# firedrakeproject/firedrake

Hardware: NVIDIA H100
Metric: assembled DoFs/sec (Poisson CG3, 256^3 hex, 1-form/action) (higher is better)
Workload: dtype f64

## Files before the change

### firedrake_b200/_lib.py

```python
from __future__ import annotations

import ctypes as C
import os

HERE = os.path.dirname(os.path.abspath(__file__))
LIB_PATH = os.environ.get("FDB200_LIB", os.path.join(HERE, "lib", "libfdb200.so"))

MAX_1D = 8

FORM_HELMHOLTZ = 1
FORM_DG_ADVECTION = 2
FORM_HELMHOLTZ_COEF = 3
FORM_NONLINEAR_DIFFUSION = 4
FORM_NONLINEAR_DIFFUSION_JACOBIAN = 5
FORM_ELASTICITY = 6
FORM_HYPERELASTICITY = 7
FORM_HYPERELASTICITY_JACOBIAN = 8
FORM_ADVECTION_DIFFUSION = 9
FORM_STOKES = 10
FORM_NAVIER_STOKES = 11
FORM_NAVIER_STOKES_JACOBIAN = 12
FORM_BOUNDARY_MASS = 13
FORM_INTERIOR_PENALTY = 14
FORM_DG_BOUNDARY = 15
# ... 20 lines not shown
    _fields_ = [
        ("form", C.c_int32), ("rank", C.c_int32), ("cell", C.c_int32),
        ("integral", C.c_int32), ("degree", C.c_int32), ("nq", C.c_int32),
        ("cdim", C.c_int32), ("scatter", C.c_int32),
        ("alpha", C.c_double), ("beta", C.c_double),
        ("B", C.c_double * (MAX_1D * MAX_1D)), ("D", C.c_double * (MAX_1D * MAX_1D)),
        ("wq", C.c_double * MAX_1D), ("xq", C.c_double * MAX_1D),
        ("offset0", C.POINTER(C.c_int32)), ("offset1", C.POINTER(C.c_int32)),
        ("diagonal", C.c_int32), ("affine_cells", C.c_int32),
        ("dcoef", C.c_double * 3),
        ("lmbda", C.c_double),
    ]


class Space2Desc(C.Structure):
    _fields_ = [
        ("degree", C.c_int32),
        ("B", C.c_double * (MAX_1D * MAX_1D)),
        ("offset", C.POINTER(C.c_int32)),
    ]


class CallArgs(C.Structure):
    _fields_ = [
        ("start", C.c_int32), ("end", C.c_int32),
        ("layers", C.POINTER(C.c_int32)), ("subset", C.c_void_p),
        ("nargs", C.c_int32), ("args", C.POINTER(C.c_void_p)),
        ("arg_bytes", C.POINTER(C.c_size_t)), ("arg_versions", C.POINTER(C.c_uint64)),
        ("nmaps", C.c_int32), ("maps", C.POINTER(C.c_void_p)),
        ("map_bytes", C.POINTER(C.c_size_t)),
        ("location", C.c_int32), ("writeback", C.c_int32), ("output_is_zero", C.c_int32),
        ("map_versions", C.POINTER(C.c_uint64)), ("subset_version", C.c_uint64),
        ("layers_count", C.c_int32), ("layers_version", C.c_uint64),
    ]


READ, WRITE, RW, INC, MIN, MAX = 1, 2, 3, 4, 5, 6
ARG_DAT, ARG_GLOBAL, ARG_MAT = 1, 2, 3
F64, F32, I32, U32, I64 = 1, 2, 3, 4, 5
REGION_ALL, REGION_ON_BOTTOM, REGION_ON_TOP, REGION_ON_INTERIOR_FACETS = 0, 1, 2, 3
WRAP_MAX_ARGS, WRAP_MAX_MAPS, WRAP_MAX_MATS = 16, 8, 4


class WrapperArg(C.Structure):
    _fields_ = [
        ("kind", C.c_int32), ("access", C.c_int32), ("dtype", C.c_int32),
        ("dim", C.c_int32), ("dim2", C.c_int32), ("map", C.c_int32), ("map2", C.c_int32),
        ("arity", C.c_int32), ("arity2", C.c_int32),
        ("offset", C.POINTER(C.c_int32)), ("offset2", C.POINTER(C.c_int32)),
        ("permutation", C.POINTER(C.c_int32)),
        ("interior_horizontal", C.c_int32),
        ("offset_quotient", C.POINTER(C.c_int32)), ("offset_quotient2", C.POINTER(C.c_int32)),
        ("mixed_continuation", C.c_int32),
    ]


class WrapperDesc(C.Structure):
    _fields_ = [
        ("kernel_source", C.c_char_p), ("kernel_name", C.c_char_p),
        ("nargs", C.c_int32), ("args", C.POINTER(WrapperArg)),
        ("extruded", C.c_int32), ("subset", C.c_int32), ("iteration_region", C.c_int32),
        ("pass_layer_arg", C.c_int32), ("extruded_periodic", C.c_int32), ("variable_layers", C.c_int32),
    ]


SIGNATURES = {
# ... 134 lines not shown
```

### firedrake_b200/csrc/action_hex.cu

```cuda
#include <stdlib.h>
#include <string.h>

#include "common.cuh"

namespace {

template <int N>
struct HelmParams {
    double *y;
    const double *x;
    const double *coords;
    const int *map0;
    const int *map1;
    const int *collist;
    const int *off0;
    const int *off1;
    int ncols;
    int col0;
    int nlay_items;
    int lay_first, lay_step;
    unsigned nlay_rcp;
    int cdim;
    const long long *rowptr;
    const int *colidx;
    double *vals;
    const int *row_lg;
    const int *col_lg;
    const unsigned short *rank_tab;
    int nvar, nlay_total;
    int chunk;
    int ws_flags;
    int *counter;
    double alpha, beta;
    double B[N * N];
    double Dt[N * N];
    double DtR[N * N];
    double DB[N * N];
    double wq[N];
    double xq[N];
};

template <int N>
struct HelmCoefParams : HelmParams<N> {
    const double *kappa;
};

template <int N>
struct HelmNlParams : HelmCoefParams<N> {
    double dcoef[3];
};

template <bool COEF>
__device__ __forceinline__ double coef_weight(double w, const double *s_kap, int q)
{
    if constexpr (COEF) return w * s_kap[q];
    else return w;
}

template <bool COEF, int NL>
__device__ __forceinline__ double stiff_weight(double w, const double *s_kap, int q, double uq, const double *dcoef)
{
    if constexpr (NL == 1) return w * fma(fma(dcoef[2], uq, dcoef[1]), uq, dcoef[0]);
    else if constexpr (NL == 2) return w;
    else return coef_weight<COEF>(w, s_kap, q);
}
// ... 258 lines not shown
    constexpr int WARPS_PER_CTA = WPC<N, SLIM, COEF>::value;
    constexpr int T = WARPS_PER_CTA * 32;
    auto kern = [] {
        if constexpr (ADV) return advection_diffusion_kernel<N, MASS, ATOMIC, MINB, MATRIX>;
        else if constexpr (NL == 1) return nonlinear_residual_kernel<N, MASS, ATOMIC, MINB, SLIM>;
        else if constexpr (NL == 2) return nonlinear_jacobian_kernel<N, MASS, ATOMIC, MINB, MATRIX, SLIM>;
        else if constexpr (COEF) return helmholtz_coef_kernel<N, MASS, ATOMIC, MINB, MATRIX, SLIM>;
        else return helmholtz_action_kernel<N, MASS, ATOMIC, MINB, MATRIX, SLIM, AFFINE>;
    }();
    static bool configured = false;
    static int occ = 1;
    if (!configured) {
        FDB_CUDA(cudaFuncSetAttribute(kern, cudaFuncAttributeMaxDynamicSharedMemorySize, WS::CTA_BYTES));
        FDB_CUDA(cudaOccupancyMaxActiveBlocksPerMultiprocessor(&occ, kern, T, WS::CTA_BYTES));
        if (occ < 1) occ = 1;
        configured = true;
    }
    const int ncells = P.ncols * P.nlay_items;
    const int nitems = (ncells + WS::CW - 1) / WS::CW;
    int per_sm = occ;
    if (grid_cap_per_sm > 0 && grid_cap_per_sm < per_sm) per_sm = grid_cap_per_sm;
    long long grid = (long long)sm_count * per_sm;
    long long need = (nitems + WARPS_PER_CTA - 1) / WARPS_PER_CTA;
    if (grid > need) grid = need;
    if (grid < 1) grid = 1;
    int chunk = P.nlay_items / WS::CW;
    if (chunk < 8) chunk = 8;
    if (chunk > 64) chunk = 64;
    long long per_warp = nitems / (grid * WARPS_PER_CTA) + 1;
    if (chunk > per_warp / 32 + 1) chunk = (int)(per_warp / 32 + 1);
    static const int chunk_env = getenv("FDB_CHUNK") ? atoi(getenv("FDB_CHUNK")) : 0;
    if (chunk_env > 0) chunk = chunk_env;
    P.chunk = chunk;
    P.nlay_rcp = (unsigned)(0x100000000ull / (unsigned long long)P.nlay_items);
    if (P.nlay_items == 1) P.nlay_rcp = 0xffffffffu;
    FDB_CUDA(cudaMemsetAsync(P.counter, 0, sizeof(int), st));
    if constexpr (NL != 0) kern<<<(int)grid, T, WS::CTA_BYTES, st>>>(P);
    else if constexpr (COEF) kern<<<(int)grid, T, WS::CTA_BYTES, st>>>(static_cast<const HelmCoefParams<N> &>(P));
    else kern<<<(int)grid, T, WS::CTA_BYTES, st>>>(static_cast<const HelmParams<N> &>(P));
    FDB_LAUNCH_CHECK();
    return 0;
}

template <int N>
struct CoefMinB {
    static constexpr int value = (N >= 5) ? 1 : 2;
};

template <int N, bool ATOMIC>
int launch_coef(bool mass, int cap, cudaStream_t st, HelmNlParams<N> &P, int sm_count)
{
    constexpr int MB = CoefMinB<N>::value;
    if (N == 6 && P.nlay_items >= 32 / N) {
        if (mass) return launch_one<N, true, ATOMIC, MB, false, (N == 6), false, true>(cap, st, P, sm_count);
        return launch_one<N, false, ATOMIC, MB, false, (N == 6), false, true>(cap, st, P, sm_count);
    }
    if (mass) return launch_one<N, true, ATOMIC, MB, false, false, false, true>(cap, st, P, sm_count);
    return launch_one<N, false, ATOMIC, MB, false, false, false, true>(cap, st, P, sm_count);
}

template <int N>
struct NlResMinB {
    static constexpr int value = (N == 4) ? 3 : ((N >= 5) ? 1 : 2);
};

template <int N, bool ATOMIC>
// ... 55 lines not shown
        constexpr bool ASL = (N == 6);
        if (!ASL || P.nlay_items >= 32 / N) {
            if (mass) return launch_one<N, true, true, AB, false, ASL, true>(cap, st, P, sm_count);
            return launch_one<N, false, true, AB, false, ASL, true>(cap, st, P, sm_count);
        }
    }
    if (N == 4 && minb == 3) {
        if (mass) return launch_one<N, true, ATOMIC, (N == 4 ? 3 : 2)>(cap, st, P, sm_count);
        return launch_one<N, false, ATOMIC, (N == 4 ? 3 : 2)>(cap, st, P, sm_count);
    }
    if (N == 4 && minb == 4) {
        if (mass) return launch_one<N, true, ATOMIC, (N == 4 ? 4 : 2)>(cap, st, P, sm_count);
        return launch_one<N, false, ATOMIC, (N == 4 ? 4 : 2)>(cap, st, P, sm_count);
    }
    if (N == 4 && minb == 1) {
        if (mass) return launch_one<N, true, ATOMIC, 1>(cap, st, P, sm_count);
        return launch_one<N, false, ATOMIC, 1>(cap, st, P, sm_count);
    }
    constexpr int DEF = (N >= 5) ? 1 : 2;
    if (N == 6) {
        static const bool slim_on = !(getenv("FDB_NO_SLIM") && atoi(getenv("FDB_NO_SLIM")));
        if (slim_on && P.nlay_items >= 32 / N) {
            if (mass) return launch_one<N, true, ATOMIC, DEF, false, (N == 6)>(cap, st, P, sm_count);
            return launch_one<N, false, ATOMIC, DEF, false, (N == 6)>(cap, st, P, sm_count);
        }
    }
    if (mass) return launch_one<N, true, ATOMIC, DEF>(cap, st, P, sm_count);
    return launch_one<N, false, ATOMIC, DEF>(cap, st, P, sm_count);
}

template <int N>
int launch_n(fdb_kernel_s *k, fdb_int start, fdb_int end, int nlay, const fdb_int *subset,
             double *y, const double *coords, const double *x, const fdb_int *map0,
             const fdb_int *map1, const double *kappa)
{
    fdb::Context &c = fdb::ctx();
    HelmNlParams<N> P;
    P.kappa = kappa;
    set_dcoef(k, P);
    const int nl = nl_mode(k);
    P.y = y;
    P.x = x;
    P.coords = coords;
    P.map0 = map0;
    P.map1 = map1;
    P.off0 = k->d_off0;
    P.off1 = k->d_off1;
    P.cdim = k->desc.cdim;
    P.alpha = k->desc.alpha;
    P.beta = k->desc.beta;
    for (int i = 0; i < N * N; i++) {
        P.B[i] = k->desc.B[i];
        P.Dt[i] = k->Dt[i];
    }
    for (int q = 0; q < N; q++)
        for (int j = 0; j < N; j++) {
            P.DtR[q * N + j] = k->Dt[q * N + (j + q) % N];
            double d = 0.0;
            for (int i = 0; i < N; i++) d += k->Dt[q * N + i] * k->desc.B[i * N + j];
            P.DB[q * N + j] = d;
        }
    for (int i = 0; i < N; i++) {
        P.wq[i] = k->desc.wq[i];
        P.xq[i] = k->desc.xq[i];
    }
    const bool mass = k->desc.beta != 0.0;
    static const int minb = getenv("FDB_MINB") ? atoi(getenv("FDB_MINB")) : 3;
    static const int cap = getenv("FDB_CTAS_PER_SM") ? atoi(getenv("FDB_CTAS_PER_SM")) : 0;
    P.counter = c.work_counter;
    if (k->desc.scatter == FDB_SCATTER_ATOMIC) {
        P.collist = subset;
        P.col0 = start;
        P.ncols = end - start;
        P.nlay_items = nlay;
        P.lay_first = 0;
        P.lay_step = 1;
        if (P.ncols <= 0 || nlay <= 0) return 0;
        if (is_adv(k)) return launch_adv<N, true>(mass, cap, c.stream, P, c.sm_count);
        if (kappa && !nl) return launch_coef<N, true>(mass, cap, c.stream, P, c.sm_count);
        if (nl) return launch_nl<N, true>(nl, mass, cap, c.stream, P, c.sm_count);
        if constexpr (N == 4) {
            static const int ws = getenv("FDB_WS") ? atoi(getenv("FDB_WS")) : 0;
            if (ws && P.cdim == 1 && nlay >= 8 && !k->desc.affine_cells) {
#define FDB_WS_CASE(id, NC, NM, NS, ST)                                                            \
    if (ws == id)                                                                              \
        return mass ? launch_ws<true, NC, NM, NS, ST>(c.stream, P, c.sm_count)                 \
                    : launch_ws<false, NC, NM, NS, ST>(c.stream, P, c.sm_count);
                FDB_WS_CASE(1, 12, 4, 2, true)
                FDB_WS_CASE(2, 8, 4, 3, true)
                FDB_WS_CASE(3, 8, 4, 3, false)
                FDB_WS_CASE(4, 8, 8, 3, false)
#undef FDB_WS_CASE
            }
        }
        return launch_variant<N, true>(mass, minb, cap, c.stream, P, c.sm_count, k->desc.affine_cells != 0);
    }
    if (subset) {
        fdb::set_error("coloured scatter does not support subsets yet");
        return 1;
    }
    for (int col = 0; col < k->ncolours; col++) {
        int cbeg = k->colour_start[col], cend = k->colour_start[col + 1];
        for (int par = 0; par < (nlay > 1 ? 2 : 1); par++) {
            P.collist = k->d_colour_cols + cbeg;
            P.col0 = 0;
            P.ncols = cend - cbeg;
            P.lay_first = par;
            P.lay_step = 2;
            P.nlay_items = (nlay - par + 1) / 2;
            if (P.ncols <= 0 || P.nlay_items <= 0) continue;
            if (is_adv(k)      ? launch_adv<N, false>(mass, cap, c.stream, P, c.sm_count)
                : kappa && !nl ? launch_coef<N, false>(mass, cap, c.stream, P, c.sm_count)
                : nl         ? launch_nl<N, false>(nl, mass, cap, c.stream, P, c.sm_count)
                             : launch_variant<N, false>(mass, minb, cap, c.stream, P, c.sm_count))
                return 1;
        }
    }
    return 0;
}

template <int N>
int launch_matrix_n(fdb_kernel_s *k, fdb_int start, fdb_int end, int nlay, const fdb_int *subset,
                    fdb_mat_t mat, const double *coords, const fdb_int *map0, const fdb_int *map1,
                    double *diag_out, const double *kappa)
{
    fdb::Context &c = fdb::ctx();
    HelmNlParams<N> P;
    memset(&P, 0, sizeof(P));
    P.kappa = kappa;
    set_dcoef(k, P);
    P.coords = coords;
    P.map0 = map0;
    P.map1 = map1;
// ... 42 lines not shown
    }
    if (nl_mode(k) == 2) {
        constexpr int MB = CoefMinB<N>::value;
        if (k->desc.beta != 0.0)
            return launch_one<N, true, true, MB, true, false, false, true, 2>(0, c.stream, P, c.sm_count);
        return launch_one<N, false, true, MB, true, false, false, true, 2>(0, c.stream, P, c.sm_count);
    }
    constexpr int DEF = (N >= 5) ? 1 : 2;
    if (k->desc.beta != 0.0) return launch_one<N, true, true, DEF, true>(0, c.stream, P, c.sm_count);
    return launch_one<N, false, true, DEF, true>(0, c.stream, P, c.sm_count);
}

}

int fdb_launch_helmholtz_matrix(fdb_kernel_s *k, fdb_int start, fdb_int end, int nlay,
                                const fdb_int *subset, fdb_mat_t mat, const double *coords,
                                const fdb_int *map0, const fdb_int *map1, double *diag_out)
{
    const int dmma = fdb_opt_matrix_kernel;
    if (mat && dmma != 0 && k->n1d <= 5 && k->n1d >= (dmma == 1 ? 3 : 4))
        return fdb_launch_helmholtz_matrix_dmma(k, start, end, nlay, subset, mat, coords, map0, map1);
    switch (k->n1d) {
    case 2: return launch_matrix_n<2>(k, start, end, nlay, subset, mat, coords, map0, map1, diag_out, nullptr);
    case 3: return launch_matrix_n<3>(k, start, end, nlay, subset, mat, coords, map0, map1, diag_out, nullptr);
    case 4: return launch_matrix_n<4>(k, start, end, nlay, subset, mat, coords, map0, map1, diag_out, nullptr);
    case 5: return launch_matrix_n<5>(k, start, end, nlay, subset, mat, coords, map0, map1, diag_out, nullptr);
    }
    fdb::set_error("helmholtz matrix: degree %d not instantiated (1..4)", k->n1d - 1);
    return 1;
}

int fdb_launch_helmholtz_action(fdb_kernel_s *k, fdb_int start, fdb_int end, int nlay,
                                const fdb_int *subset, double *y, const double *coords,
                                const double *x, const fdb_int *map0, const fdb_int *map1)
{
    static const bool q1_thread = !(getenv("FDB_Q1_THREAD") && atoi(getenv("FDB_Q1_THREAD")) == 0);
    if (q1_thread && k->n1d == 2 && k->desc.cdim == 1 && k->desc.scatter == FDB_SCATTER_ATOMIC &&
        k->desc.cell == FDB_CELL_HEX_EXTRUDED && nlay >= 16)
        return fdb_launch_q1_action(k, start, end, nlay, subset, y, coords, x, map0, map1);
    static const bool q2_thread = !(getenv("FDB_Q2_THREAD") && atoi(getenv("FDB_Q2_THREAD")) == 0);
    if (q2_thread && k->n1d == 3 && k->desc.cdim == 1 && k->desc.scatter == FDB_SCATTER_ATOMIC &&
        k->desc.cell == FDB_CELL_HEX_EXTRUDED && nlay >= 16)
        return fdb_launch_q2_action(k, start, end, nlay, subset, y, coords, x, map0, map1);
    switch (k->n1d) {
    case 2: return launch_n<2>(k, start, end, nlay, subset, y, coords, x, map0, map1, nullptr);
    case 3: return launch_n<3>(k, start, end, nlay, subset, y, coords, x, map0, map1, nullptr);
    case 4: return launch_n<4>(k, start, end, nlay, subset, y, coords, x, map0, map1, nullptr);
    case 5: return launch_n<5>(k, start, end, nlay, subset, y, coords, x, map0, map1, nullptr);
    case 6: return launch_n<6>(k, start, end, nlay, subset, y, coords, x, map0, map1, nullptr);
    }
    fdb::set_error("helmholtz action: degree %d not instantiated (1..5)", k->n1d - 1);
    return 1;
}

int fdb_launch_helmholtz_coef_action(fdb_kernel_s *k, fdb_int start, fdb_int end, int nlay,
                                     const fdb_int *subset, double *y, const double *coords,
                                     const double *x, const double *kappa, const fdb_int *map0,
                                     const fdb_int *map1)
{
    switch (k->n1d) {
    case 2: return launch_n<2>(k, start, end, nlay, subset, y, coords, x, map0, map1, kappa);
    case 3: return launch_n<3>(k, start, end, nlay, subset, y, coords, x, map0, map1, kappa);
    case 4: return launch_n<4>(k, start, end, nlay, subset, y, coords, x, map0, map1, kappa);
    case 5: return launch_n<5>(k, start, end, nlay, subset, y, coords, x, map0, map1, kappa);
    case 6: return launch_n<6>(k, start, end, nlay, subset, y, coords, x, map0, map1, kappa);
    }
    fdb::set_error("helmholtz_coef action: degree %d not instantiated (1..5)", k->n1d - 1);
    return 1;
}

int fdb_launch_helmholtz_coef_matrix(fdb_kernel_s *k, fdb_int start, fdb_int end, int nlay,
                                     const fdb_int *subset, fdb_mat_t mat, const double *coords,
                                     const double *kappa, const fdb_int *map0, const fdb_int *map1,
                                     double *diag_out)
{
    switch (k->n1d) {
    case 2: return launch_matrix_n<2>(k, start, end, nlay, subset, mat, coords, map0, map1, diag_out, kappa);
    case 3: return launch_matrix_n<3>(k, start, end, nlay, subset, mat, coords, map0, map1, diag_out, kappa);
    case 4: return launch_matrix_n<4>(k, start, end, nlay, subset, mat, coords, map0, map1, diag_out, kappa);
    case 5: return launch_matrix_n<5>(k, start, end, nlay, subset, mat, coords, map0, map1, diag_out, kappa);
    }
    fdb::set_error("helmholtz_coef matrix: degree %d not instantiated (1..4)", k->n1d - 1);
// ... 3 lines not shown
```

### firedrake_b200/csrc/action_hex_body.cuh

```cuda
    static_assert(!(SLIM && MATRIX), "matrix mode keeps the per-cell index buffer");
    static_assert(!(AFFINE && MATRIX), "the affine variant exists for 1-forms only");
    static_assert(!(AFFINE && COEF), "the coefficient form has no affine variant");
    static_assert(NL != 1 || (!COEF && !MATRIX && !AFFINE), "the residual is a 1-form without a kappa buffer");
    static_assert(NL != 2 || (COEF && !AFFINE), "the Jacobian keeps u in the kappa buffer");
    static_assert(!ADV || (COEF && NL == 0 && !SLIM && !AFFINE), "b takes the coefficient layout, three times");
    using WS = WarpSmem<N, SLIM, COEF, ADV ? 3 : 1>;
    constexpr int CW = WS::CW;
    constexpr int CWS = WS::CWS;
    constexpr int ND = N * N * N;
    constexpr int US = WS::US;
    constexpr int CS = WS::CS;
    extern __shared__ __align__(16) unsigned char smem_raw[];
    const int lane = threadIdx.x & 31, warp = threadIdx.x >> 5;
    double *wbase = reinterpret_cast<double *>(smem_raw + (size_t)warp * WS::BYTES);
    double *s_tile = wbase;
    double *s_u = s_tile + WS::TILE;
    double *s_coord = s_u + WS::UBUF;
    double *s_stash = s_coord + WS::COORD;
    constexpr bool STASH = WS::STASH > 0 && !MATRIX && !AFFINE;
    double *s_kap = s_stash + WS::STASH;
    int *s_idx = reinterpret_cast<int *>(s_kap + WS::KAPPA);
    int *s_mapraw = s_idx + WS::IDX;
    int *s_vidx = s_mapraw + WS::MAPRAW;
    int *s_off0 = reinterpret_cast<int *>(smem_raw + (size_t)WPC<N, SLIM, COEF>::value * WS::BYTES);
// ... 134 lines not shown
                const int loc = j * N + t;
                const int g = SLIM ? sm[loc] + s_off0[loc] * u.layer : si[loc];
                if constexpr (ADV) {
#pragma unroll
                    for (int c = 0; c < 3; c++) cp_async8(sk + c * WS::UBUF + loc, kappa + 3ll * g + c);
                } else {
                    cp_async8(sk + loc, kappa + g);
                }
            }
        }
    };

    Unit cur{-1, 0, 0, 0, 0, false, 0, 0, 0, false};
    cur = advance(cur);
    decode(cur);
    Unit nxt = advance(cur);
    decode(nxt);
    stageA(cur);
    cp_async_commit();
    cp_async_wait<0>();
    __syncwarp();
    int ubuf = 0;
    stageB_coords(cur);
#pragma unroll
    for (int part = 0; part < N; part++) stageB_part(cur, ubuf, part);
    stageB_kappa(cur);
    stageA(nxt);
    cp_async_commit();
    double A1[3], A3[3], A6[3], c2[3], c4[3], c5[3], c7[3];
    double Gm[6], adet_c = 1.0;
#pragma unroll
    for (int i = 0; i < 6; i++) Gm[i] = 0.0;

    while (cur.item >= 0) {
        cp_async_wait<0>();
        __syncwarp();
        Unit nn = advance(nxt);
        decode(nn);

        const bool valid = cur.valid;
        const int cbuf = cur.ib;
        const double *sc = s_coord + cw * CS;
        if (cur.comp == 0) {
#pragma unroll
            for (int a = 0; a < 3; a++) {
                double X000 = sc[0 * 3 + a], X001 = sc[1 * 3 + a], X010 = sc[2 * 3 + a],
                       X011 = sc[3 * 3 + a], X100 = sc[4 * 3 + a], X101 = sc[5 * 3 + a],
                       X110 = sc[6 * 3 + a], X111 = sc[7 * 3 + a];
                if (!valid) {
                    X000 = 0; X001 = (a == 2); X010 = (a == 1); X011 = (a >= 1);
                    X100 = (a == 0); X101 = (a != 1); X110 = (a != 2); X111 = 1;
                }
                double c1 = X100 - X000;
                c2[a] = X010 - X000;
                double c3 = X001 - X000;
                c4[a] = X110 - X100 - X010 + X000;
                c5[a] = X011 - X010 - X001 + X000;
                double c6 = X101 - X100 - X001 + X000;
                c7[a] = X111 - X110 - X101 - X011 + X100 + X010 + X001 - X000;
                A1[a] = fma(c4[a], eta, c1);
                A3[a] = fma(c5[a], eta, c3);
                A6[a] = fma(c7[a], eta, c6);
            }
            if (AFFINE) {
                double r0[3], r1[3], r2[3];
                r0[0] = c2[1] * A3[2] - c2[2] * A3[1];
                r0[1] = c2[2] * A3[0] - c2[0] * A3[2];
                r0[2] = c2[0] * A3[1] - c2[1] * A3[0];
                r1[0] = A3[1] * A1[2] - A3[2] * A1[1];
                r1[1] = A3[2] * A1[0] - A3[0] * A1[2];
                r1[2] = A3[0] * A1[1] - A3[1] * A1[0];
// ... 315 lines not shown
```

### firedrake_b200/csrc/common.cuh

```cuda
#pragma once
#include <cuda_runtime.h>
#include <stdint.h>
#include <stdio.h>
#include <string.h>

#include <string>

#include "../../include/fdb200.h"

namespace fdb {

struct Context {
    bool ready = false;
    int device = -1;
    int sm_count = 0;
    cudaStream_t stream = nullptr;
    uint64_t launches = 0;
    void *flush_buf = nullptr;
    size_t flush_bytes = 0;
    double *reduce_scratch = nullptr;
    double *reduce_host = nullptr;
    int *work_counter = nullptr;
};

// ... 63 lines not shown
typedef struct fdb_mat_s *fdb_mat_t;
int fdb_mat_device_view(fdb_mat_t m, const long long **rowptr, const fdb_int **colidx, double **vals,
                        const fdb_int **row_lg, const fdb_int **col_lg);
int fdb_mat_rank_table(fdb_mat_t m, const unsigned short **rank, int *nvar);
int fdb_mat_block_size(fdb_mat_t m, int *bs);
int fdb_mat_rows(fdb_mat_t m, fdb_int *nrows);
int fdb_mat_scalar_view_begin(fdb_mat_t blocked, fdb_mat_t *view);
int fdb_mat_scalar_view_end(fdb_mat_t blocked, fdb_mat_t view);
int fdb_launch_helmholtz_matrix(fdb_kernel_s *k, fdb_int start, fdb_int end, int nlay,
                                const fdb_int *subset, fdb_mat_t mat, const double *coords,
                                const fdb_int *map0, const fdb_int *map1, double *diag_out);

int fdb_launch_helmholtz_matrix_dmma(fdb_kernel_s *k, fdb_int start, fdb_int end, int nlay,
                                     const fdb_int *subset, fdb_mat_t mat, const double *coords,
                                     const fdb_int *map0, const fdb_int *map1);

int fdb_launch_tri_p1(fdb_kernel_s *k, fdb_int start, fdb_int end, const fdb_int *subset, double *y,
                      const double *coords, const double *x, const fdb_int *map, fdb_mat_t mat);
int fdb_launch_dg_advection(fdb_kernel_s *k, fdb_int start, fdb_int end, const fdb_int *subset,
                            double *out, const double *coords, const double *q, const double *u,
                            const double *consts_host, const unsigned *facet, const fdb_int *dgmap,
                            const fdb_int *cgmap, const fdb_int *nbr);

int fdb_launch_q1_action(fdb_kernel_s *k, fdb_int start, fdb_int end, int nlay, const fdb_int *subset,
                         double *y, const double *coords, const double *x, const fdb_int *map0,
                         const fdb_int *map1);

int fdb_launch_q2_action(fdb_kernel_s *k, fdb_int start, fdb_int end, int nlay, const fdb_int *subset,
                         double *y, const double *coords, const double *x, const fdb_int *map0,
                         const fdb_int *map1);

int fdb_launch_helmholtz_action(fdb_kernel_s *k, fdb_int start, fdb_int end, int nlay,
                                const fdb_int *subset, double *y, const double *coords,
                                const double *x, const fdb_int *map0, const fdb_int *map1);
int fdb_launch_helmholtz_coef_action(fdb_kernel_s *k, fdb_int start, fdb_int end, int nlay,
                                     const fdb_int *subset, double *y, const double *coords,
                                     const double *x, const double *kappa, const fdb_int *map0,
                                     const fdb_int *map1);
int fdb_launch_helmholtz_coef_matrix(fdb_kernel_s *k, fdb_int start, fdb_int end, int nlay,
                                     const fdb_int *subset, fdb_mat_t mat, const double *coords,
                                     const double *kappa, const fdb_int *map0, const fdb_int *map1,
                                     double *diag_out);
int fdb_launch_elasticity_action(fdb_kernel_s *k, fdb_int start, fdb_int end, int nlay, const fdb_int *subset,
                                 double *y, const double *coords, const double *x, const double *u,
                                 const fdb_int *map0, const fdb_int *map1);
int fdb_launch_elasticity_matrix(fdb_kernel_s *k, fdb_int start, fdb_int end, int nlay, const fdb_int *subset,
                                 fdb_mat_t mat, const double *coords, const double *u, const fdb_int *map0,
                                 const fdb_int *map1, double *diag_out);
int fdb_launch_stokes_action(fdb_kernel_s *k, fdb_int start, fdb_int end, int nlay, const fdb_int *subset,
                             double *yu, const double *coords, const double *u, double *yp, const double *p,
                             const double *ulin, const fdb_int *map0, const fdb_int *map1, const fdb_int *map2);
int fdb_launch_boundary_mass(fdb_kernel_s *k, fdb_int start, fdb_int end, int nlay, const fdb_int *subset,
                             fdb_mat_t mat, double *y, const double *coords, const double *x, const unsigned *facet,
                             const fdb_int *map0, const fdb_int *map1);
int fdb_launch_dg_facet(fdb_kernel_s *k, fdb_int start, fdb_int end, int nlay, const fdb_int *subset, double *y,
                        const double *coords, const double *x, const unsigned *facet, const fdb_int *map0,
                        const fdb_int *map1);
int fdb_launch_dg_transport(fdb_kernel_s *k, fdb_int start, fdb_int end, int nlay, const fdb_int *subset, double *y,
                            const double *coords, const double *x, const double *b, const unsigned *facet,
                            const fdb_int *map0, const fdb_int *map1);
int fdb_launch_dg_upwind(fdb_kernel_s *k, fdb_int start, fdb_int end, int nlay, const fdb_int *subset, double *y,
                         const double *coords, const double *x, const double *b, const unsigned *facet,
                         const fdb_int *map0, const fdb_int *map1);
```

### firedrake_b200/csrc/global_kernel.cu

```cuda
#include <math.h>
#include <stdlib.h>
#include <string.h>

#include <algorithm>
#include <vector>

#include "common.cuh"

using namespace fdb;

namespace {

int collocated_derivative(int n, const double *B, const double *D, double *Dt)
{
    double A[FDB_MAX_1D][FDB_MAX_1D], R[FDB_MAX_1D][FDB_MAX_1D];
    for (int i = 0; i < n; i++)
        for (int j = 0; j < n; j++) {
            A[i][j] = B[j * n + i];
            R[i][j] = D[j * n + i];
        }
    for (int c = 0; c < n; c++) {
        int piv = c;
        for (int r = c + 1; r < n; r++)
            if (fabs(A[r][c]) > fabs(A[piv][c])) piv = r;
// ... 601 lines not shown
            return 1;
        }
    }
    if (f->coef && f->coef_cdim != k->desc.cdim && a->location == FDB_LOC_HOST && a->arg_bytes && mode != MODE_DIAGONAL) {
        size_t nodes;
        if (mat) {
            fdb_int rows = 0;
            fdb_mat_rows(mat, &rows);
            nodes = (size_t)rows;
        } else {
            nodes = a->arg_bytes[2] / (sizeof(double) * k->desc.cdim);
        }
        if (a->arg_bytes[want - 1] < nodes * f->coef_cdim * sizeof(double)) {
            set_error("fdb_kernel_call: %s %s: %s has %d values per node, %zu bytes are too few for %zu nodes",
                      f->name, mode_name[mode], f->coef, f->coef_cdim, a->arg_bytes[want - 1], nodes);
            return 1;
        }
    }
    if (f->launcher == LAUNCH_HELMHOLTZ && mode == MODE_ACTION && a->location == FDB_LOC_HOST && a->arg_versions &&
        a->arg_bytes && a->map_bytes && a->writeback && a->output_is_zero && !a->subset && extruded &&
        k->desc.scatter == FDB_SCATTER_ATOMIC) {
        int rc = pipelined_host_action(k, a, nlay);
        if (rc >= 0) return rc;
    }
    void *dargs[6];
    const fdb_int *dmaps[3];
    const fdb_int *dsubset;
    if (device_pointers(a, mat != nullptr, dargs, dmaps, &dsubset)) return 1;
    const double *coords = (const double *)dargs[1];
    const double *coef = f->coef ? (const double *)dargs[want - 1] : nullptr;
    const double *vel = f->launcher == LAUNCH_DG_TRANSPORT ? (const double *)dargs[mode == MODE_ACTION ? 3 : 2] : nullptr;
    const unsigned *tfacets = transport_facets ? (const unsigned *)dargs[want - 1] : nullptr;
    double *out = mat ? nullptr : (double *)dargs[0];
    if (mode != MODE_ACTION) {
        switch (f->launcher) {
        case LAUNCH_HELMHOLTZ:
            if (mat && k->desc.cdim > 1) {
                fdb_mat_t view = nullptr;
                if (fdb_mat_scalar_view_begin(mat, &view)) return 1;
                int rc = fdb_launch_helmholtz_matrix(k, a->start, a->end, nlay, dsubset, view, coords, dmaps[0],
                                                     dmaps[1], nullptr);
                int rc2 = fdb_mat_scalar_view_end(mat, view);
                return rc ? rc : rc2;
            }
            return fdb_launch_helmholtz_matrix(k, a->start, a->end, nlay, dsubset, mat, coords, dmaps[0], dmaps[1],
                                               out);
        case LAUNCH_HELMHOLTZ_COEF:
            return fdb_launch_helmholtz_coef_matrix(k, a->start, a->end, nlay, dsubset, mat, coords, coef, dmaps[0],
                                                    dmaps[1], out);
        case LAUNCH_BOUNDARY:
            return fdb_launch_boundary_mass(k, a->start, a->end, nlay, dsubset, mat, out, coords, nullptr,
                                            (const unsigned *)coef, dmaps[0], dmaps[1]);
        case LAUNCH_DG_FACET:
            return fdb_launch_dg_facet(k, a->start, a->end, nlay, dsubset, out, coords, nullptr,
                                       (const unsigned *)coef, dmaps[0], dmaps[1]);
        case LAUNCH_DG_TRANSPORT:
            return fdb_launch_dg_transport(k, a->start, a->end, nlay, dsubset, out, coords, nullptr, vel, tfacets,
                                           dmaps[0], dmaps[1]);
        default:
            return fdb_launch_elasticity_matrix(k, a->start, a->end, nlay, dsubset, mat, coords, coef, dmaps[0],
                                                dmaps[1], out);
        }
    }
    if (k->desc.scatter == FDB_SCATTER_COLOURED && !(f->launcher == LAUNCH_DG_TRANSPORT && !transport_facets) &&
        (k->colour_map_key != (const void *)a->maps[0] || k->colour_map_gen != map_ver(a, 0) ||
         k->colour_end != a->end)) {
        std::vector<fdb_int> hmap;
        const fdb_int *src = a->maps[0];
        if (a->location == FDB_LOC_DEVICE) {
            hmap.resize((size_t)a->end * k->arity);
            FDB_CUDA(cudaMemcpy(hmap.data(), a->maps[0], sizeof(fdb_int) * hmap.size(),
                                cudaMemcpyDeviceToHost));
            src = hmap.data();
        }
        if (build_colouring(k, src, a->end)) return 1;
        k->colour_map_key = (const void *)a->maps[0];
        k->colour_map_gen = map_ver(a, 0);
        k->colour_end = a->end;
    }
    if (k->desc.scatter == FDB_SCATTER_COLOURED && a->start != 0) {
        set_error("fdb_kernel_call: coloured scatter needs start == 0");
        return 1;
    }
    const double *x = (const double *)dargs[2];
    int rc;
    switch (f->launcher) {
    case LAUNCH_HELMHOLTZ:
        rc = fdb_launch_helmholtz_action(k, a->start, a->end, nlay, dsubset, out, coords, x, dmaps[0], dmaps[1]);
        break;
    case LAUNCH_HELMHOLTZ_COEF:
        rc = fdb_launch_helmholtz_coef_action(k, a->start, a->end, nlay, dsubset, out, coords, x, coef, dmaps[0],
                                              dmaps[1]);
        break;
    case LAUNCH_ELASTICITY:
        rc = fdb_launch_elasticity_action(k, a->start, a->end, nlay, dsubset, out, coords, x, coef, dmaps[0],
                                          dmaps[1]);
        break;
    case LAUNCH_BOUNDARY:
        rc = fdb_launch_boundary_mass(k, a->start, a->end, nlay, dsubset, nullptr, out, coords, x,
                                      (const unsigned *)coef, dmaps[0], dmaps[1]);
        break;
    case LAUNCH_DG_FACET:
        rc = fdb_launch_dg_facet(k, a->start, a->end, nlay, dsubset, out, coords, x, (const unsigned *)coef,
                                 dmaps[0], dmaps[1]);
        break;
    case LAUNCH_DG_TRANSPORT:
        rc = fdb_launch_dg_transport(k, a->start, a->end, nlay, dsubset, out, coords, x, vel, tfacets, dmaps[0],
                                     dmaps[1]);
        break;
    default:
        rc = fdb_launch_stokes_action(k, a->start, a->end, nlay, dsubset, out, coords, x, (double *)dargs[3],
                                      (const double *)dargs[4], coef, dmaps[0], dmaps[1], dmaps[2]);
    }
    if (rc) return rc;
    if (a->location == FDB_LOC_HOST && a->writeback) {
        if (fdb_mirror_writeback(a->args[0])) return 1;
        if (a->arg_versions) fdb_mirror_set_version(a->args[0], a->arg_versions[0] + 1);
    }
    return 0;
}

// ... 2 lines not shown
```

### firedrake_b200/op2.py

```python
from __future__ import annotations

import ctypes as C
import enum
import itertools
import weakref
from dataclasses import dataclass, field
from typing import NamedTuple

import numpy as np

from . import _lib
from ._lib import EngineError

IntType = np.int32
ScalarType = np.float64


class Access(enum.IntEnum):
    READ = 1
    WRITE = 2
    RW = 3
    INC = 4
    MIN = 5
    MAX = 6
# ... 402 lines not shown
        return self

    def __isub__(self, other):
        self.axpy(-1.0, other)
        return self

    def __imul__(self, scalar):
        for d in self._dats:
            d.__imul__(scalar)
        return self


class Dat:
    _ids = itertools.count()
    zero_rotation = False

    def __init__(self, dataset, data=None, dtype=ScalarType, name=None, pinned=False):
        self.dataset = _as_dataset(dataset)
        shape = (self.dataset.set.total_size,) + (self.dataset.dim if self.dataset.cdim > 1 else ())
        self._pinned = None
        if pinned:
            self._pinned = PinnedArray(shape, dtype)
            self._data = self._pinned.array
            self._data[...] = 0 if data is None else np.asarray(data, dtype=dtype).reshape(shape)
        elif data is None:
            self._data = np.zeros(shape, dtype=dtype)
        else:
            self._data = np.ascontiguousarray(np.asarray(data, dtype=dtype).reshape(shape))
        self.dtype = np.dtype(dtype)
        self.name = name or f"dat_{next(Dat._ids)}"
        self.dat_version = 0
        self._dev = None
        self._spare = None
        self._host_valid = True
        self._dev_valid = False
        self._is_zero = data is None
        self.halo_valid = True
        self.frozen_halo = False

    @property
    def cdim(self):
        return self.dataset.cdim

    @property
    def nbytes(self):
        return self._data.nbytes

    def _sync_host(self):
        if not self._host_valid:
            if self._is_zero:
                self._data[...] = 0
            else:
                self._dev.to_host(self._data)
            self._host_valid = True

    @property
    def data_ro(self):
        self._sync_host()
        v = self._data[:self.dataset.set.size].view()
        v.setflags(write=False)
        return v

    @property
    def data_ro_with_halos(self):
        self._sync_host()
        v = self._data.view()
# ... 32 lines not shown
        self.increment_dat_version()
        self._dev_valid = False
        self._is_zero = False
        return self._data

    def increment_dat_version(self):
        self.dat_version += 1

    def split(self):
        return (self,)

    def __iter__(self):
        yield self

    def __len__(self):
        return 1

    def __getitem__(self, i):
        if i != 0:
            raise IndexError("a Dat has the block 0 only")
        return self

    def save(self, filename):
        np.save(filename, self.data_ro)

    def load(self, filename):
        import os
        if not os.path.exists(filename) and os.path.exists(str(filename) + ".npy"):
            filename = str(filename) + ".npy"
        v = np.load(filename)
        if v.shape != self._data[:self.dataset.set.size].shape:
            raise ValueError("file holds an array of a different shape")
        self.data_wo[...] = v

    @property
    def device_ptr(self):
        if self._dev is None:
            self._dev = DeviceArray(self._data.nbytes)
        if not self._dev_valid:
            if self._is_zero:
                _lib.check(_lib.lib().fdb_memset(self._dev.ptr, 0, self._data.nbytes), "memset")
            else:
                _lib.check(_lib.lib().fdb_memcpy_h2d(self._dev.ptr, self._data.ctypes.data,
                                                     self._data.nbytes), "h2d")
            self._dev_valid = True
        return self._dev.ptr

    def _device_written(self, halo_valid=False):
        self._host_valid = False
        self._dev_valid = True
        self._is_zero = False
        self.halo_valid = bool(halo_valid)
        self.increment_dat_version()

    def _reset_ghost_rows(self, access):
        st = self.dataset.set
        nghost = (st.total_size - st.size) * self.cdim
        if nghost <= 0 or (self._is_zero and access is INC):
            return
        ident = {INC: 0.0, MIN: float("inf"), MAX: float("-inf")}[access]
        base = self.device_ptr + st.size * self.cdim * self.dtype.itemsize
        _lib.check(_lib.lib().fdb_vec_fill(nghost, ident, base), "fdb_vec_fill")

    def zero(self, subset=None):
        if subset is not None:
            if self._dev_valid and not self._host_valid:
                if not hasattr(subset, "_dev_idx"):
                    subset._dev_idx = DeviceArray.from_host(subset.indices)
                _lib.check(_lib.lib().fdb_dat_zero_nodes(self._dev.ptr, self.cdim, subset._dev_idx.ptr,
                                                         len(subset.indices)), "zero_nodes")
                self.increment_dat_version()
            else:
                self.data_with_halos[subset.indices] = 0
            return
        self._host_valid = False
        self._dev_valid = False
        self._is_zero = True
        self.increment_dat_version()
        if self._dev is not None and Dat.zero_rotation:
            L = _lib.lib()
            if self._spare is None:
                self._spare = DeviceArray(self._data.nbytes)
                _lib.check(L.fdb_zero_background(self._spare.ptr, self._data.nbytes))
            _lib.check(L.fdb_background_barrier())
            self._dev, self._spare = self._spare, self._dev
            _lib.check(L.fdb_zero_background(self._spare.ptr, self._data.nbytes))
            self._dev_valid = True

    def _vec_op(self, other, fn, *scalars):
        L = _lib.lib()
        n = self._data.size
        _lib.check(fn(n, *scalars, other.device_ptr, self.device_ptr))
        self._device_written(halo_valid=self.halo_valid and other.halo_valid)

    def axpy(self, alpha, other):
        self._vec_op(other, _lib.lib().fdb_vec_axpy, float(alpha))

    def inner(self, other):
        out = C.c_double()
        _lib.check(_lib.lib().fdb_vec_dot(self._data.size, self.device_ptr, other.device_ptr,
                                          C.byref(out)), "dot")
        return out.value

    def norm(self):
        return float(np.sqrt(self.inner(self)))

# ... 769 lines not shown
                        s2.B[q * lk.degree + a] = elq.B[q, a]
        for q in range(el.nq):
            d.wq[q] = el.wq[q]
            d.xq[q] = el.xq[q]
            for a in range(n):
                d.B[q * n + a] = el.B[q, a]
                d.D[q * n + a] = el.D[q, a]
        m0, m1 = self.arguments[:2]
        keep = []
        if self.extruded:
            if m0.offset is None or m1.offset is None:
                raise MapValueError("extruded parloop needs maps with offsets")
            o0 = np.ascontiguousarray(m0.offset, dtype=IntType)
            o1 = np.ascontiguousarray(m1.offset, dtype=IntType)
            keep = [o0, o1]
            d.offset0 = o0.ctypes.data_as(C.POINTER(C.c_int32))
            d.offset1 = o1.ctypes.data_as(C.POINTER(C.c_int32))
            if spec.pressure and len(self.arguments) > 2 and self.arguments[2].offset is not None:
                o2 = np.ascontiguousarray(self.arguments[2].offset, dtype=IntType)
                keep.append(o2)
                s2.offset = o2.ctypes.data_as(C.POINTER(C.c_int32))
        h = C.c_void_p()
        if s2 is not None:
            _lib.check(_lib.lib().fdb_kernel_create_mixed(C.byref(d), C.byref(s2), C.byref(h)),
                       "fdb_kernel_create_mixed")
        else:
            _lib.check(_lib.lib().fdb_kernel_create(C.byref(d), C.byref(h)), "fdb_kernel_create")
        del keep
        self._handle = h
        return h

    def __call__(self, start, end, layers, subset_indices, args, arg_bytes, arg_versions,
                 maps, map_bytes, location, writeback, output_is_zero, map_versions=None,
                 subset_version=0):
        h = self.compile()
        ca = _lib.CallArgs()
        ca.start, ca.end = int(start), int(end)
        if layers is not None:
            ca.layers = layers.ctypes.data_as(C.POINTER(C.c_int32))
        ca.subset = subset_indices
        ca.nargs = len(args)
        ca.args = (C.c_void_p * len(args))(*args)
        if arg_bytes is not None:
            ca.arg_bytes = (C.c_size_t * len(args))(*arg_bytes)
            ca.arg_versions = (C.c_uint64 * len(args))(*arg_versions)
        ca.nmaps = len(maps)
        ca.maps = (C.c_void_p * len(maps))(*maps)
        if map_bytes is not None:
            ca.map_bytes = (C.c_size_t * len(maps))(*map_bytes)
        if map_versions is not None:
            ca.map_versions = (C.c_uint64 * len(maps))(*map_versions)
        ca.subset_version = int(subset_version)
        ca.location = location
        ca.writeback = int(writeback)
        ca.output_is_zero = int(output_is_zero)
        _lib.check(_lib.lib().fdb_kernel_call(h, C.byref(ca)), self.name)

    def __del__(self):
        try:
            if self._handle is not None and _lib._initialised is not None:
                _lib._lib.fdb_kernel_destroy(self._handle)
        except Exception:
            pass


class _PhaseTimer:
    _inst = None

    def __init__(self, on):
        self.on, self.t, self.acc = on, None, {}
        if on:
            import atexit
            atexit.register(self.report)

    @classmethod
    def get(cls):
        if cls._inst is None:
            import os
            cls._inst = cls(os.environ.get("FDB_PHASE_TIMING") == "1")
        if cls._inst.on:
            import time
            _lib.check(_lib.lib().fdb_synchronize())
            cls._inst.t = time.perf_counter()
        return cls._inst

    def mark(self, name):
        if self.on:
            import time
# ... 25 lines not shown
            raise NotImplementedError("periodic extrusion (offset_quotient) runs on the generic wrapper path: "
                                      "pass the local kernel as C source (op2.Kernel(code, name))")
        if not getattr(base, "constant_layers", True):
            raise NotImplementedError("variable layers run on the generic wrapper path: "
                                      "pass the local kernel as C source (op2.Kernel(code, name))")
        lk = self.global_kernel.local_kernel
        if len(self.args) != len(lk.accesses):
            raise ValueError(f"kernel takes {len(lk.accesses)} arguments, got {len(self.args)}")
        spec = _FORMS.get(getattr(lk, "form", None))
        if spec and spec.coef_cdim and self.args[-1].data.cdim != spec.coef_cdim:
            raise ValueError(f"{lk.form}: the trailing coefficient has {spec.coef_cdim} values per node, "
                             f"{self.args[-1].data.name} has {self.args[-1].data.cdim}")
        if spec and spec.velocity:
            b = self.args[2 if lk.diagonal else 3]
            if b.data.cdim != 3 or b.map is not self.args[1].map:
                raise ValueError(f"{lk.form}: b has 3 values per vertex and is read through the coordinate map, "
                                 f"{b.data.name} has {b.data.cdim} through {getattr(b.map, 'name', None)}")
        if spec and spec.pressure:
            for a in self.args[3:5]:
                if a.data.cdim != 1:
                    raise ValueError(f"{lk.form}: the pressure Dats have 1 value per node, {a.data.name} has "
                                     f"{a.data.cdim}")
        for a, acc in zip(self.args, lk.accesses):
            if a.access != acc:
                raise ValueError(f"argument {a.data.name}: access {a.access.name} != kernel's {acc.name}")
            if a.map is not None:
                base = self.iterset.superset if isinstance(self.iterset, Subset) else self.iterset
                if a.map.iterset is not base:
                    raise MapValueError(f"map {a.map.name} is not defined on the iteration set")
                toset = (a.data.sparsity.dsets[0].set if isinstance(a.data, Mat)
                         else a.data.dataset.set)
                if a.map.toset is not toset:
                    raise MapValueError(f"map {a.map.name} does not target {a.data.name}'s set")

    def _compute(self, part):
        start, end = part
        if end <= start:
            return
        gk = self.global_kernel
        it = self.iterset
        layers = it.layers_array.ravel() if it._extruded else None
        out = self.args[0].data
        maps = []
        for a in self.args:
            if a.map is not None and a.map not in maps:
                maps.append(a.map)
        if isinstance(out, Mat):
            L = _lib.lib()
            lg = self.args[0].lgmaps
            if lg is not None:
                r, c = (np.ascontiguousarray(v, dtype=IntType) for v in lg)
                _lib.check(L.fdb_mat_set_lgmaps(out.handle, r.ctypes.data, c.ctypes.data))
            subset = None
            if isinstance(it, Subset):
                if not hasattr(it, "_dev_idx"):
                    it._dev_idx = DeviceArray.from_host(it.indices)
                subset = it._dev_idx.ptr
            ins = [a.data.device_ptr for a in self.args[1:]]
            try:
                gk(start, end, layers, subset, [out.handle.value] + ins, None, None,
                   [m.device_ptr for m in maps], None, _lib.LOC_DEVICE, False, False)
            finally:
                if lg is not None:
                    _lib.check(L.fdb_mat_set_lgmaps(out.handle, None, None))
            out.dat_version += 1
            return
        if self.location == "device":
            subset = None
            if isinstance(it, Subset):
                if not hasattr(it, "_dev_idx"):
                    it._dev_idx = DeviceArray.from_host(it.indices)
                subset = it._dev_idx.ptr
            ptrs = [a.data._data.ctypes.data if isinstance(a.data, Global) else a.data.device_ptr
                    for a in self.args]
            gk(start, end, layers, subset, ptrs, None, None, [m.device_ptr for m in maps], None,
               _lib.LOC_DEVICE, False, False)
            out._device_written()
            for a in self.args[1:]:
                if a.access == INC:
                    a.data._device_written()
        else:
            subset = it.indices.ctypes.data if isinstance(it, Subset) else None
            lazy_zero = out._is_zero and not out._host_valid
            for a in self.args:
                if not (a.data is out and lazy_zero):
                    a.data._sync_host()
            ptrs = [a.data._data.ctypes.data for a in self.args]
            nbytes = [a.data._data.nbytes for a in self.args]
            vers = [a.data.dat_version for a in self.args]
            gk(start, end, layers, subset, ptrs, nbytes, vers,
               [m.values_with_halo.ctypes.data for m in maps],
               [m.values_with_halo.nbytes for m in maps], _lib.LOC_HOST, True, out._is_zero,
               map_versions=[m._generation for m in maps],
               subset_version=it._generation if isinstance(it, Subset) else 0)
            out.increment_dat_version()
            out._is_zero = False
            out._host_valid = True
            out._dev_valid = False

    def __call__(self):
        reads = [a.data for a in self.args
                 if a.access == READ and isinstance(a.data, Dat) and a.data.dataset.halo is not None
                 and not a.data.halo_valid]
        if reads and self.location != "device":
            base0 = self.iterset.superset if isinstance(self.iterset, Subset) else self.iterset
            if getattr(base0, "owner_computes", False) and len(self.args) == 3 and not isinstance(self.iterset, Subset):
                return self._call_host_partitioned()
            raise NotImplementedError("halo exchanges on host-resident Dats need an exec-halo partition "
                                      "(SlabPartition(exec_halo=True)); otherwise use location='device'")
        incs = [a.data for a in self.args
# ... 133 lines not shown
```

### include/fdb200.h

```cpp
#ifndef FDB200_H
#define FDB200_H

#include <stddef.h>
#include <stdint.h>

#ifdef __cplusplus
extern "C" {
#endif

typedef int32_t fdb_int;

int fdb_init(int device);
int fdb_finalize(void);
const char *fdb_last_error(void);
int fdb_synchronize(void);
int fdb_device_info(char *name, int name_len, int *sm_count, size_t *total_mem);
uint64_t fdb_launch_count(void);

int fdb_set_option(const char *name, int value);
int fdb_get_option(const char *name, int *value);

void *fdb_malloc(size_t nbytes);
int fdb_free(void *dptr);
int fdb_memset(void *dptr, int value, size_t nbytes);
// ... 85 lines not shown
    const fdb_int *offset;
} fdb_space2_desc;

typedef struct fdb_kernel_s *fdb_kernel_t;

int fdb_kernel_create(const fdb_kernel_desc *desc, fdb_kernel_t *out);
int fdb_kernel_create_mixed(const fdb_kernel_desc *desc, const fdb_space2_desc *space2, fdb_kernel_t *out);
int fdb_kernel_destroy(fdb_kernel_t k);

int fdb_cells_are_affine(const double *coords, const fdb_int *map1, const fdb_int *off1_host,
                         fdb_int start, fdb_int end, int nlay, int *result);

#define FDB_LOC_HOST 0
#define FDB_LOC_DEVICE 1

typedef struct fdb_call_args {
    fdb_int start, end;
    const fdb_int *layers;
    const fdb_int *subset;
    int32_t nargs;
    void *const *args;
    const size_t *arg_bytes;
    const uint64_t *arg_versions;
    int32_t nmaps;
    const fdb_int *const *maps;
    const size_t *map_bytes;
    int32_t location;
    int32_t writeback;
    int32_t output_is_zero;
    const uint64_t *map_versions;
    uint64_t subset_version;
    fdb_int layers_count;
    uint64_t layers_version;
} fdb_call_args;

int fdb_kernel_call(fdb_kernel_t k, const fdb_call_args *a);

enum fdb_access { FDB_READ = 1, FDB_WRITE = 2, FDB_RW = 3, FDB_INC = 4, FDB_MIN = 5, FDB_MAX = 6 };
enum fdb_arg_kind { FDB_ARG_DAT = 1, FDB_ARG_GLOBAL = 2, FDB_ARG_MAT = 3 };
enum fdb_dtype { FDB_F64 = 1, FDB_F32 = 2, FDB_I32 = 3, FDB_U32 = 4, FDB_I64 = 5 };
enum fdb_region {
    FDB_REGION_ALL = 0, FDB_REGION_ON_BOTTOM = 1, FDB_REGION_ON_TOP = 2,
    FDB_REGION_ON_INTERIOR_FACETS = 3
};

#define FDB_WRAP_MAX_ARGS 16
#define FDB_WRAP_MAX_MAPS 8
#define FDB_WRAP_MAX_MATS 4

typedef struct fdb_wrapper_arg {
    int32_t kind;
    int32_t access;
    int32_t dtype;
    int32_t dim;
    int32_t dim2;
    int32_t map;
    int32_t map2;
    int32_t arity, arity2;
    const fdb_int *offset;
    const fdb_int *offset2;
    const fdb_int *permutation;
    int32_t interior_horizontal;
    const fdb_int *offset_quotient;
    const fdb_int *offset_quotient2;
    int32_t mixed_continuation;
} fdb_wrapper_arg;
// ... 86 lines not shown
```

Before: 34.08 billion.

## Zero the output twin buffer inside the action kernel for the next call

Adds a double-buffered twin for large output Dats. Each action launch zeroes the spare buffer as a side task inside the kernel, using streaming stores striped across work items. The next zero() then swaps buffers instead of issuing a separate memset. This removes a standalone memset pass over the output between repeated assemblies, at the cost of doubled device memory for the output, extra store traffic inside the compute kernel, and more complex state tracking.

```diff
diff --git a/firedrake_b200/_lib.py b/firedrake_b200/_lib.py
--- a/firedrake_b200/_lib.py
+++ b/firedrake_b200/_lib.py
@@ -76,6 +76,7 @@
         ("location", C.c_int32), ("writeback", C.c_int32), ("output_is_zero", C.c_int32),
         ("map_versions", C.POINTER(C.c_uint64)), ("subset_version", C.c_uint64),
         ("layers_count", C.c_int32), ("layers_version", C.c_uint64),
+        ("zero_next", C.c_void_p), ("zero_next_bytes", C.c_size_t),
     ]
 
 
diff --git a/firedrake_b200/csrc/action_hex.cu b/firedrake_b200/csrc/action_hex.cu
--- a/firedrake_b200/csrc/action_hex.cu
+++ b/firedrake_b200/csrc/action_hex.cu
@@ -31,6 +31,9 @@
     int chunk;
     int ws_flags;
     int *counter;
+    double2 *zero_next;
+    long long zero_next_n2;
+    int zero_next_stripe;
     double alpha, beta;
     double B[N * N];
     double Dt[N * N];
@@ -355,6 +358,10 @@
     static const int chunk_env = getenv("FDB_CHUNK") ? atoi(getenv("FDB_CHUNK")) : 0;
     if (chunk_env > 0) chunk = chunk_env;
     P.chunk = chunk;
+    if (P.zero_next) {
+        const long long stripe = (P.zero_next_n2 + nitems - 1) / nitems;
+        P.zero_next_stripe = (int)((stripe + 31) / 32 * 32);
+    }
     P.nlay_rcp = (unsigned)(0x100000000ull / (unsigned long long)P.nlay_items);
     if (P.nlay_items == 1) P.nlay_rcp = 0xffffffffu;
     FDB_CUDA(cudaMemsetAsync(P.counter, 0, sizeof(int), st));
@@ -476,13 +483,16 @@
 template <int N>
 int launch_n(fdb_kernel_s *k, fdb_int start, fdb_int end, int nlay, const fdb_int *subset,
              double *y, const double *coords, const double *x, const fdb_int *map0,
-             const fdb_int *map1, const double *kappa)
+             const fdb_int *map1, const double *kappa, void *zero_next = nullptr, size_t zero_next_bytes = 0)
 {
     fdb::Context &c = fdb::ctx();
     HelmNlParams<N> P;
     P.kappa = kappa;
     set_dcoef(k, P);
     const int nl = nl_mode(k);
+    P.zero_next = nullptr;
+    P.zero_next_n2 = 0;
+    P.zero_next_stripe = 0;
     P.y = y;
     P.x = x;
     P.coords = coords;
@@ -519,13 +529,25 @@
         P.nlay_items = nlay;
         P.lay_first = 0;
         P.lay_step = 1;
+        static const int ws = (N == 4 && getenv("FDB_WS")) ? atoi(getenv("FDB_WS")) : 0;
+        const bool take_ws = ws && P.cdim == 1 && nlay >= 8 && !k->desc.affine_cells;
+        if (zero_next) {
+            if (P.ncols > 0 && nlay > 0 && !is_adv(k) && !kappa && !nl && !take_ws && !k->desc.affine_cells) {
+                P.zero_next = (double2 *)zero_next;
+                P.zero_next_n2 = (long long)(zero_next_bytes / sizeof(double2));
+                if (zero_next_bytes % sizeof(double2))
+                    FDB_CUDA(cudaMemsetAsync((char *)zero_next + zero_next_bytes - sizeof(double), 0, sizeof(double),
+                                             c.stream));
+            } else {
+                FDB_CUDA(cudaMemsetAsync(zero_next, 0, zero_next_bytes, c.stream));
+            }
+        }
         if (P.ncols <= 0 || nlay <= 0) return 0;
         if (is_adv(k)) return launch_adv<N, true>(mass, cap, c.stream, P, c.sm_count);
         if (kappa && !nl) return launch_coef<N, true>(mass, cap, c.stream, P, c.sm_count);
         if (nl) return launch_nl<N, true>(nl, mass, cap, c.stream, P, c.sm_count);
         if constexpr (N == 4) {
-            static const int ws = getenv("FDB_WS") ? atoi(getenv("FDB_WS")) : 0;
-            if (ws && P.cdim == 1 && nlay >= 8 && !k->desc.affine_cells) {
+            if (take_ws) {
 #define FDB_WS_CASE(id, NC, NM, NS, ST)                                                            \
     if (ws == id)                                                                              \
         return mass ? launch_ws<true, NC, NM, NS, ST>(c.stream, P, c.sm_count)                 \
@@ -543,6 +565,7 @@
         fdb::set_error("coloured scatter does not support subsets yet");
         return 1;
     }
+    if (zero_next) FDB_CUDA(cudaMemsetAsync(zero_next, 0, zero_next_bytes, c.stream));
     for (int col = 0; col < k->ncolours; col++) {
         int cbeg = k->colour_start[col], cend = k->colour_start[col + 1];
         for (int par = 0; par < (nlay > 1 ? 2 : 1); par++) {
@@ -651,22 +674,25 @@
 
 int fdb_launch_helmholtz_action(fdb_kernel_s *k, fdb_int start, fdb_int end, int nlay,
                                 const fdb_int *subset, double *y, const double *coords,
-                                const double *x, const fdb_int *map0, const fdb_int *map1)
+                                const double *x, const fdb_int *map0, const fdb_int *map1, void *zero_next,
+                                size_t zero_next_bytes)
 {
     static const bool q1_thread = !(getenv("FDB_Q1_THREAD") && atoi(getenv("FDB_Q1_THREAD")) == 0);
-    if (q1_thread && k->n1d == 2 && k->desc.cdim == 1 && k->desc.scatter == FDB_SCATTER_ATOMIC &&
-        k->desc.cell == FDB_CELL_HEX_EXTRUDED && nlay >= 16)
-        return fdb_launch_q1_action(k, start, end, nlay, subset, y, coords, x, map0, map1);
     static const bool q2_thread = !(getenv("FDB_Q2_THREAD") && atoi(getenv("FDB_Q2_THREAD")) == 0);
-    if (q2_thread && k->n1d == 3 && k->desc.cdim == 1 && k->desc.scatter == FDB_SCATTER_ATOMIC &&
-        k->desc.cell == FDB_CELL_HEX_EXTRUDED && nlay >= 16)
+    const bool thread_per_cell = k->desc.cdim == 1 && k->desc.scatter == FDB_SCATTER_ATOMIC &&
+                                 k->desc.cell == FDB_CELL_HEX_EXTRUDED && nlay >= 16 &&
+                                 ((q1_thread && k->n1d == 2) || (q2_thread && k->n1d == 3));
+    if (thread_per_cell) {
+        if (zero_next) FDB_CUDA(cudaMemsetAsync(zero_next, 0, zero_next_bytes, fdb::ctx().stream));
+        if (k->n1d == 2) return fdb_launch_q1_action(k, start, end, nlay, subset, y, coords, x, map0, map1);
         return fdb_launch_q2_action(k, start, end, nlay, subset, y, coords, x, map0, map1);
+    }
     switch (k->n1d) {
-    case 2: return launch_n<2>(k, start, end, nlay, subset, y, coords, x, map0, map1, nullptr);
-    case 3: return launch_n<3>(k, start, end, nlay, subset, y, coords, x, map0, map1, nullptr);
-    case 4: return launch_n<4>(k, start, end, nlay, subset, y, coords, x, map0, map1, nullptr);
-    case 5: return launch_n<5>(k, start, end, nlay, subset, y, coords, x, map0, map1, nullptr);
-    case 6: return launch_n<6>(k, start, end, nlay, subset, y, coords, x, map0, map1, nullptr);
+    case 2: return launch_n<2>(k, start, end, nlay, subset, y, coords, x, map0, map1, nullptr, zero_next, zero_next_bytes);
+    case 3: return launch_n<3>(k, start, end, nlay, subset, y, coords, x, map0, map1, nullptr, zero_next, zero_next_bytes);
+    case 4: return launch_n<4>(k, start, end, nlay, subset, y, coords, x, map0, map1, nullptr, zero_next, zero_next_bytes);
+    case 5: return launch_n<5>(k, start, end, nlay, subset, y, coords, x, map0, map1, nullptr, zero_next, zero_next_bytes);
+    case 6: return launch_n<6>(k, start, end, nlay, subset, y, coords, x, map0, map1, nullptr, zero_next, zero_next_bytes);
     }
     fdb::set_error("helmholtz action: degree %d not instantiated (1..5)", k->n1d - 1);
     return 1;
diff --git a/firedrake_b200/csrc/action_hex_body.cuh b/firedrake_b200/csrc/action_hex_body.cuh
--- a/firedrake_b200/csrc/action_hex_body.cuh
+++ b/firedrake_b200/csrc/action_hex_body.cuh
@@ -190,11 +190,20 @@
 #pragma unroll
     for (int i = 0; i < 6; i++) Gm[i] = 0.0;
 
+    constexpr bool ZNEXT = ATOMIC && !AFFINE && !COEF && NL == 0 && !ADV && !MATRIX;
+
     while (cur.item >= 0) {
         cp_async_wait<0>();
         __syncwarp();
         Unit nn = advance(nxt);
         decode(nn);
+        if constexpr (ZNEXT) {
+            if (P.zero_next && cur.comp == 0) {
+                const long long s0 = (long long)cur.item * P.zero_next_stripe + lane;
+                for (int k = 0; k < P.zero_next_stripe; k += 32)
+                    if (s0 + k < P.zero_next_n2) __stcs(P.zero_next + s0 + k, make_double2(0.0, 0.0));
+            }
+        }
 
         const bool valid = cur.valid;
         const int cbuf = cur.ib;
diff --git a/firedrake_b200/csrc/common.cuh b/firedrake_b200/csrc/common.cuh
--- a/firedrake_b200/csrc/common.cuh
+++ b/firedrake_b200/csrc/common.cuh
@@ -119,7 +119,8 @@
 
 int fdb_launch_helmholtz_action(fdb_kernel_s *k, fdb_int start, fdb_int end, int nlay,
                                 const fdb_int *subset, double *y, const double *coords,
-                                const double *x, const fdb_int *map0, const fdb_int *map1);
+                                const double *x, const fdb_int *map0, const fdb_int *map1,
+                                void *zero_next = nullptr, size_t zero_next_bytes = 0);
 int fdb_launch_helmholtz_coef_action(fdb_kernel_s *k, fdb_int start, fdb_int end, int nlay,
                                      const fdb_int *subset, double *y, const double *coords,
                                      const double *x, const double *kappa, const fdb_int *map0,
diff --git a/firedrake_b200/csrc/global_kernel.cu b/firedrake_b200/csrc/global_kernel.cu
--- a/firedrake_b200/csrc/global_kernel.cu
+++ b/firedrake_b200/csrc/global_kernel.cu
@@ -657,6 +657,15 @@
     const double *vel = f->launcher == LAUNCH_DG_TRANSPORT ? (const double *)dargs[mode == MODE_ACTION ? 3 : 2] : nullptr;
     const unsigned *tfacets = transport_facets ? (const unsigned *)dargs[want - 1] : nullptr;
     double *out = mat ? nullptr : (double *)dargs[0];
+    void *zero_next = a->location == FDB_LOC_DEVICE ? a->zero_next : nullptr;
+    if (zero_next && a->zero_next_bytes % sizeof(double)) {
+        set_error("fdb_kernel_call: zero_next_bytes (%zu) is not a multiple of 8", a->zero_next_bytes);
+        return 1;
+    }
+    if (zero_next && !(f->launcher == LAUNCH_HELMHOLTZ && mode == MODE_ACTION)) {
+        FDB_CUDA(cudaMemsetAsync(zero_next, 0, a->zero_next_bytes, ctx().stream));
+        zero_next = nullptr;
+    }
     if (mode != MODE_ACTION) {
         switch (f->launcher) {
         case LAUNCH_HELMHOLTZ:
@@ -711,7 +720,8 @@
     int rc;
     switch (f->launcher) {
     case LAUNCH_HELMHOLTZ:
-        rc = fdb_launch_helmholtz_action(k, a->start, a->end, nlay, dsubset, out, coords, x, dmaps[0], dmaps[1]);
+        rc = fdb_launch_helmholtz_action(k, a->start, a->end, nlay, dsubset, out, coords, x, dmaps[0], dmaps[1],
+                                         zero_next, zero_next ? a->zero_next_bytes : 0);
         break;
     case LAUNCH_HELMHOLTZ_COEF:
         rc = fdb_launch_helmholtz_coef_action(k, a->start, a->end, nlay, dsubset, out, coords, x, coef, dmaps[0],
diff --git a/firedrake_b200/op2.py b/firedrake_b200/op2.py
--- a/firedrake_b200/op2.py
+++ b/firedrake_b200/op2.py
@@ -458,6 +458,8 @@
         self.dat_version = 0
         self._dev = None
         self._spare = None
+        self._twin = None
+        self._twin_zero = False
         self._host_valid = True
         self._dev_valid = False
         self._is_zero = data is None
@@ -556,6 +558,13 @@
         if v.shape != self._data[:self.dataset.set.size].shape:
             raise ValueError("file holds an array of a different shape")
         self.data_wo[...] = v
+
+    def _twin_to_zero(self):
+        if self._twin_zero or self._dev is None or Dat.zero_rotation:
+            return None
+        if self._twin is None:
+            self._twin = DeviceArray(self._data.nbytes)
+        return self._twin.ptr
 
     @property
     def device_ptr(self):
@@ -596,6 +605,14 @@
                 self.increment_dat_version()
             else:
                 self.data_with_halos[subset.indices] = 0
+            return
+        if self._twin_zero and self._dev is not None:
+            self._dev, self._twin = self._twin, self._dev
+            self._twin_zero = False
+            self._host_valid = False
+            self._dev_valid = True
+            self._is_zero = True
+            self.increment_dat_version()
             return
         self._host_valid = False
         self._dev_valid = False
@@ -1431,7 +1448,7 @@
 
     def __call__(self, start, end, layers, subset_indices, args, arg_bytes, arg_versions,
                  maps, map_bytes, location, writeback, output_is_zero, map_versions=None,
-                 subset_version=0):
+                 subset_version=0, zero_next=None, zero_next_bytes=0):
         h = self.compile()
         ca = _lib.CallArgs()
         ca.start, ca.end = int(start), int(end)
@@ -1453,6 +1470,8 @@
         ca.location = location
         ca.writeback = int(writeback)
         ca.output_is_zero = int(output_is_zero)
+        if zero_next is not None:
+            ca.zero_next, ca.zero_next_bytes = zero_next, int(zero_next_bytes)
         _lib.check(_lib.lib().fdb_kernel_call(h, C.byref(ca)), self.name)
 
     def __del__(self):
@@ -1544,6 +1563,14 @@
                          else a.data.dataset.set)
                 if a.map.toset is not toset:
                     raise MapValueError(f"map {a.map.name} does not target {a.data.name}'s set")
+
+    twin_min_bytes = 64 << 20
+
+    def _zeroes_twin(self, out):
+        lk = self.global_kernel.local_kernel
+        return (isinstance(out, Dat) and out.nbytes >= self.twin_min_bytes and self.global_kernel.extruded
+                and getattr(lk, "form", None) == "helmholtz" and getattr(lk, "rank", 0) == 1
+                and not getattr(lk, "diagonal", False) and self.global_kernel.scatter == "atomic")
 
     def _compute(self, part):
         start, end = part
@@ -1585,9 +1612,12 @@
                 subset = it._dev_idx.ptr
             ptrs = [a.data._data.ctypes.data if isinstance(a.data, Global) else a.data.device_ptr
                     for a in self.args]
+            twin = out._twin_to_zero() if self._zeroes_twin(out) else None
             gk(start, end, layers, subset, ptrs, None, None, [m.device_ptr for m in maps], None,
-               _lib.LOC_DEVICE, False, False)
+               _lib.LOC_DEVICE, False, False, zero_next=twin, zero_next_bytes=out.nbytes)
             out._device_written()
+            if twin is not None:
+                out._twin_zero = True
             for a in self.args[1:]:
                 if a.access == INC:
                     a.data._device_written()
diff --git a/include/fdb200.h b/include/fdb200.h
--- a/include/fdb200.h
+++ b/include/fdb200.h
@@ -141,6 +141,8 @@
     uint64_t subset_version;
     fdb_int layers_count;
     uint64_t layers_version;
+    void *zero_next;
+    size_t zero_next_bytes;
 } fdb_call_args;
 
 int fdb_kernel_call(fdb_kernel_t k, const fdb_call_args *a);
```

New measurement: 34.78 billion (median of 6 runs). +2.0%, better.
